# manuelbb-upb/Morbit.jl

Hardware: AMD Instinct MI355X
Metric: RBF build+solve+eval cycles/sec (higher is better)
Workload: dtype f64

## Files before the change

include/mrbf.h:

```cpp
#ifndef MRBF_H
#define MRBF_H

#include <stdint.h>

#ifdef __cplusplus
extern "C" {
#endif

typedef struct mrbf_ctx mrbf_ctx;
typedef struct mrbf_model mrbf_model;

enum {
    MRBF_CUBIC = 0,
    MRBF_INV_MULTIQUADRIC = 1,
    MRBF_MULTIQUADRIC = 2,
    MRBF_THIN_PLATE_SPLINE = 3,
    MRBF_GAUSSIAN = 4
};

enum {
    MRBF_OK = 0,
    MRBF_ENOTPD = 1,
    MRBF_ESINGULAR = 2,
    MRBF_EHIP = 3,
// ... 169 lines not shown

int32_t mrbf_debug_env(const char *name);
int32_t mrbf_debug_mfma_layout(mrbf_ctx *ctx, double *out16x16_a_times_b, const double *A16x4, const double *B4x16);
int32_t mrbf_debug_potrf(mrbf_ctx *ctx, int64_t n, double *A_colmajor_inout, int32_t impl, int32_t *info, float *ms);
int32_t mrbf_debug_diag(mrbf_ctx *ctx, const double *A128, int32_t reps, float *ms_per_call, double *shader_cycles,
                        double *realtime_us);
int32_t mrbf_debug_mfma_peak(mrbf_ctx *ctx, int32_t blocks_per_cu, int32_t threads, int32_t iters, float *ms, double *tflops);
int32_t mrbf_debug_mfma_asm(mrbf_ctx *ctx, int32_t variant, int32_t blocks_per_cu, int32_t iters, float *ms, double *tflops,
                            double *cycles_per_mfma);
int32_t mrbf_debug_dgemm(mrbf_ctx *ctx, int32_t m, int32_t n, int32_t k, float *ms, double *tflops);
int32_t mrbf_debug_mega_tables(int32_t nt, int32_t mt, int32_t slack, int32_t slack_chain, int32_t first, int32_t win, int32_t srows,
                               int32_t half_cols, int64_t *out6);
int32_t mrbf_debug_mega_tables2(int32_t nt, int32_t mt, int32_t slack, int32_t slack_chain, int32_t first, int32_t win, int32_t srows,
                                int32_t half_cols, const int32_t *opt5, int64_t *out6);
int32_t mrbf_debug_mega_plan(int32_t nt, int32_t mt, int32_t xreal, int64_t *out39);

enum { MRBF_PS_OK = 0, MRBF_PS_CRITICAL = 1, MRBF_PS_FAILURE = 2 };
typedef struct {
    int32_t max_ideal_evals;
    int32_t max_ps_evals;
    int32_t max_polish_evals;
    int32_t reserved;
    uint64_t seed;
    double t0;
    double xtol_rel;
} mrbf_ps_options;
typedef struct {
    int32_t status;
    int32_t generations;
    int32_t evals_ideal, evals_ps, evals_polish;
// ... 135 lines not shown
```

morbit.jl_amd/_lib.py:

```python
import ctypes
import os

import numpy as np

_HERE = os.path.dirname(os.path.abspath(__file__))
LIB_PATH = os.environ.get("MRBF_LIB") or os.path.join(_HERE, "libmrbf.so")

c_dp = ctypes.POINTER(ctypes.c_double)
c_fp = ctypes.POINTER(ctypes.c_float)
c_ip = ctypes.POINTER(ctypes.c_int32)
c_vp = ctypes.c_void_p

MRBF_OK, MRBF_ENOTPD, MRBF_ESINGULAR, MRBF_EHIP, MRBF_EBLAS, MRBF_ENOMEM, MRBF_ENODEVICE, MRBF_ENCCL = range(8)
PATH_CHOL, PATH_PROJ_CHOL, PATH_LU, PATH_MINNORM, PATH_ROUND4 = 1, 2, 3, 4, 5
OPT_GRAM_MODE, OPT_RESIDUAL, OPT_FORCE_PATH, OPT_CHOL_IMPL, OPT_EVAL_IMPL, OPT_TIMING, OPT_DIAG_IMPL, OPT_CHOL_WINDOW = 1, 2, 3, 4, 5, 6, 7, 8
OPT_SPIN_MS, OPT_DEBUG_FAULT, OPT_LAST_DEVICE_MS, OPT_SLOW_LAUNCHES = 9, 10, 11, 12
OPT_ARENA_BYTES, OPT_LIVE_HANDLES = 13, 14
FB_CHOL_HOST_DRIVEN, FB_BACKSOLVE_BLOCKED, FB_LU = 1, 2, 4


class FitInfo(ctypes.Structure):
    _fields_ = [("path", ctypes.c_int32), ("factor_info", ctypes.c_int32), ("n", ctypes.c_int32), ("q", ctypes.c_int32),
                ("rel_residual", ctypes.c_double), ("max_pitw", ctypes.c_double), ("mu", ctypes.c_double),
                ("ms_gram", ctypes.c_float), ("ms_project", ctypes.c_float), ("ms_factor", ctypes.c_float),
# ... 167 lines not shown
    "mrbf_batch_run": (ctypes.c_int32, [ctypes.c_int32, c_ip, ctypes.c_int64, ctypes.POINTER(Problem),
                                        ctypes.POINTER(Result)]),
    "mrbf_fit_batch": (ctypes.c_int32, [c_vp, ctypes.c_int64, ctypes.POINTER(FitJob), c_fp]),
    "mrbf_dispatch_fit_batch": (ctypes.c_int32, [ctypes.c_int64]),
    "mrbf_debug_mfma_layout": (ctypes.c_int32, [c_vp, c_vp, c_vp, c_vp]),
    "mrbf_debug_potrf": (ctypes.c_int32, [c_vp, ctypes.c_int64, c_vp, ctypes.c_int32, c_ip, c_fp]),
    "mrbf_debug_env": (ctypes.c_int32, [ctypes.c_char_p]),
    "mrbf_debug_diag": (ctypes.c_int32, [c_vp, c_vp, ctypes.c_int32, c_fp, c_dp, c_dp]),
    "mrbf_debug_ps_rank": (ctypes.c_int32, [c_vp, ctypes.c_int32, c_vp, c_vp, ctypes.c_uint64, ctypes.c_int32, ctypes.c_int32, c_ip, c_ip]),
    "mrbf_debug_mfma_peak": (ctypes.c_int32, [c_vp, ctypes.c_int32, ctypes.c_int32, ctypes.c_int32, c_fp, c_dp]),
    "mrbf_debug_mfma_asm": (ctypes.c_int32, [c_vp, ctypes.c_int32, ctypes.c_int32, ctypes.c_int32, c_fp, c_dp, c_dp]),
    "mrbf_debug_dgemm": (ctypes.c_int32, [c_vp, ctypes.c_int32, ctypes.c_int32, ctypes.c_int32, c_fp, c_dp]),
    "mrbf_debug_mega_tables": (ctypes.c_int32, [ctypes.c_int32] * 8 + [c_vp]),
    "mrbf_debug_mega_tables2": (ctypes.c_int32, [ctypes.c_int32] * 8 + [c_vp, c_vp]),
    "mrbf_debug_mega_plan": (ctypes.c_int32, [ctypes.c_int32] * 3 + [c_vp]),
    "mrbf_stochastic_rank": (ctypes.c_int32, [ctypes.c_int32, c_vp, c_vp, c_vp, ctypes.c_double, c_vp]),
    "mrbf_ps_step": (ctypes.c_int32, [c_vp, c_vp, c_vp, c_vp, c_vp, c_vp, c_vp, ctypes.POINTER(PsOptions), c_vp, c_vp, c_vp,
                                      ctypes.POINTER(PsInfo)]),
    "mrbf_ps_step_problem": (ctypes.c_int32, [c_vp, ctypes.POINTER(PsProblem), c_vp, c_vp, c_vp, c_vp, c_vp, ctypes.POINTER(PsOptions),
                                              c_vp, c_vp, c_vp, ctypes.POINTER(PsInfo)]),
    "mrbf_ps_step_batch": (ctypes.c_int32, [c_vp, ctypes.c_int64, ctypes.POINTER(PsProblem), ctypes.POINTER(ctypes.c_void_p), c_vp, c_vp, c_vp,
                                            c_vp, c_vp, ctypes.POINTER(PsOptions), ctypes.POINTER(ctypes.c_uint64), c_vp, c_vp, c_vp,
                                            ctypes.POINTER(PsInfo), c_fp]),
    "mrbf_dispatch_ps_batch": (ctypes.c_int32, [ctypes.c_int64] + [ctypes.c_int32] * 6),
    "mrbf_sd_direction": (ctypes.c_int32, [c_vp, ctypes.c_int64, ctypes.c_int32, ctypes.c_int32, ctypes.c_int32, ctypes.c_int32] + [c_vp] * 8
                          + [ctypes.c_int32, c_vp, c_vp, c_vp, c_vp, c_vp]),
    "mrbf_sd_criticality": (ctypes.c_int32, [c_vp, ctypes.POINTER(PsProblem), c_vp, c_vp, c_vp, c_vp, ctypes.c_int32, c_vp, c_vp,
                                             ctypes.POINTER(SdInfo)]),
    "mrbf_normal_direction": (ctypes.c_int32, [c_vp, ctypes.c_int64, ctypes.c_int32, ctypes.c_int32, ctypes.c_int32] + [c_vp] * 12),
    "mrbf_normal_step": (ctypes.c_int32, [c_vp, ctypes.POINTER(PsProblem), ctypes.c_int32, c_vp, c_vp, c_vp, ctypes.c_double, ctypes.c_double,
# ... 112 lines not shown
```

morbit.jl_amd/csrc/batch.hip:

```cpp
#include <algorithm>
#include <thread>

#include "common.hpp"
#include "small.hpp"

namespace mrbf {

int batch_run_chain(int n_dev, const int *devs, const std::vector<int64_t> &which, const mrbf_problem *problems, mrbf_result *results);
mrbf_ctx *batch_pool_acquire(int device, int *rc);
void batch_pool_release(mrbf_ctx *c);
void fill_small_prob(const mrbf_ctx *ctx, const mrbf_model *M, const double *Y, double *ws, int *flags, double *scal, int *cl, smallfit::Prob *P);
int small_fit_verdict(const mrbf_model *M, const int *hflags, const double *hscal, mrbf_fit_info *info);
int check_kernel(mrbf_ctx *ctx, int kid, double a, double b, int deg, int argpos);

struct CheckDesc {
    const double *V, *Y;
    const double *C, *Wc, *W;
    const double *vals;
    int64_t n, npad, m;
    int d, k, q;
    double *out;
};

__global__ __launch_bounds__(256) void batch_check_kernel(const CheckDesc *__restrict__ many, int part) {
// ... 103 lines not shown
    if (longest == 0) return 0;
    const unsigned gx = (unsigned)std::min<int64_t>((longest + 2047) / 2048, 256);
    hipLaunchKernelGGL(batch_copy_kernel, dim3(gx, (unsigned)count), dim3(256), 0, ctx->stream, dsegs);
    MRBF_HIP(ctx, hipGetLastError());
    return 0;
}

static int run_small_batch(mrbf_ctx *ctx, const std::vector<int64_t> &idx, const mrbf_problem *problems, mrbf_result *results,
                           std::vector<int64_t> *redo, int force_nc = 0, const mrbf_model *keep = nullptr, float *ms_sum = nullptr) {
    const int P = (int)idx.size();
    if (P == 0) return 0;
    (void)hipSetDevice(ctx->device);
    struct Lay {
        size_t C, Y, X, Xc, sq, mean, W, Wc, lam, ws, Xq0, xsq0, vp0, gp0, V0, Xq1, xsq1, vp1, gp1, vals, jac, out;
        int nsplit0, nsplit1, D, q, KO;
        int64_t npad, mpad0, mpad1;
        bool w_host, lam_host;
    };
    std::vector<Lay> lay(P);
    size_t total = 0;
    auto take = [&](size_t cnt) {
        const size_t at = total;
        total += al16(std::max<size_t>(cnt, 1));
        return at;
    };
    const bool check = ctx->residual != 0;
    const size_t out0 = take((size_t)10 * P);
    for (int i = 0; i < P; ++i) {
        const mrbf_problem &pr = problems[idx[i]];
        Lay &L = lay[i];
// ... 8 lines not shown
        L.X = (pr.m == 0 || is_device_ptr(pr.X)) ? (size_t)-1 : take((size_t)pr.m * d);
        const bool w_dev = pr.weights_out && is_device_ptr(pr.weights_out), lam_dev = pr.poly_out && L.q > 0 && is_device_ptr(pr.poly_out);
        L.w_host = pr.weights_out && !w_dev;
        L.lam_host = pr.poly_out && L.q > 0 && !lam_dev;
        L.Xc = L.sq = L.mean = L.W = L.Wc = L.lam = (size_t)-1;
        if (!keep) {
            L.Xc = take((size_t)L.npad * L.D);
            L.sq = take((size_t)L.npad);
            L.mean = take((size_t)L.D);
            if (!w_dev) L.W = take((size_t)pr.n * k);
            L.Wc = take((size_t)L.npad * k);
            if (!lam_dev) L.lam = take((size_t)std::max(L.q, 1) * k);
        }
        L.ws = take(smallfit::carve((int)L.npad, q16).total);
        L.mpad0 = check ? round_up(pr.n, 64) : 0;
        L.nsplit0 = check ? eval_nsplit(ctx, pr.n, (int)((pr.n + 63) / 64), true) : 1;
        L.Xq0 = take((size_t)L.mpad0 * L.D);
        L.xsq0 = take((size_t)L.mpad0);
        L.vp0 = take(L.nsplit0 > 1 ? (size_t)L.nsplit0 * L.mpad0 * L.KO * 2 : 0);
        L.gp0 = take((size_t)0);
        L.V0 = take((size_t)pr.n * k);
        L.mpad1 = round_up(pr.m, 64);
        L.nsplit1 = pr.m > 0 ? eval_nsplit(ctx, pr.m, (int)((pr.n + 63) / 64)) : 1;
        L.Xq1 = take((size_t)L.mpad1 * L.D);
        L.xsq1 = take((size_t)L.mpad1);
        L.vp1 = take(L.nsplit1 > 1 ? (size_t)L.nsplit1 * L.mpad1 * L.KO * 2 : 0);
        L.gp1 = take((pr.jac_out && L.nsplit1 > 1) ? (size_t)L.nsplit1 * L.mpad1 * L.KO * L.D : 0);
        L.vals = (pr.m == 0 || (pr.vals_out && is_device_ptr(pr.vals_out))) ? (size_t)-1 : take((size_t)pr.m * k);
        L.jac = (pr.m == 0 || !pr.jac_out || is_device_ptr(pr.jac_out)) ? (size_t)-1 : take((size_t)pr.m * k * d);
        L.out = out0 + (size_t)8 * i;
    }
    const size_t arena_budget = (size_t)(mrbf_env("MRBF_BATCH_ARENA_MB") ? atoll(mrbf_env("MRBF_BATCH_ARENA_MB")) : 8192) << 20;
    auto halves = [&]() -> int {
        const std::vector<int64_t> lo(idx.begin(), idx.begin() + P / 2), hi(idx.begin() + P / 2, idx.end());
        MRBF_TRY(run_small_batch(ctx, lo, problems, results, redo, force_nc, keep, ms_sum));
        return run_small_batch(ctx, hi, problems, results, redo, force_nc, keep, ms_sum);
    };
    if (P > 1 && total * sizeof(double) > arena_budget) return halves();
// ... 66 lines not shown
            M.lam = K.lam;
            if (pr.weights_out && !L.w_host) segs[(size_t)P + i] = CopySeg{M.W, pr.weights_out, pr.n * pr.k};
            if (pr.poly_out && L.q > 0 && !L.lam_host) segs[(size_t)2 * P + i] = CopySeg{M.lam, pr.poly_out, (int64_t)L.q * pr.k};
        } else {
            M.Xc = base + L.Xc;
            M.sq = base + L.sq;
            M.mean = base + L.mean;
            M.W = L.W == (size_t)-1 ? pr.weights_out : base + L.W;
            M.Wc = base + L.Wc;
            M.lam = L.lam == (size_t)-1 ? pr.poly_out : base + L.lam;
        }
        fill_small_prob(ctx, &M, Y, base + L.ws, flags + 4 * i, base + L.out + 5, dcl + smallfit::CL_WORDS * i, &probs[i]);
        probs[i].mean_given = 1;
        for (int e = 0; e < 2; ++e) {
            EvalDesc &E = evs[(size_t)e * P + i];
            eval_desc_model(E, &M, e == 0 ? (check ? pr.n : 0) : pr.m, e == 0 ? L.nsplit0 : L.nsplit1);
            E.X = e == 0 ? C : X;
            E.Xq = base + (e == 0 ? L.Xq0 : L.Xq1);
            E.xsq = base + (e == 0 ? L.xsq0 : L.xsq1);
            E.vpart = base + (e == 0 ? L.vp0 : L.vp1);
            E.sapart = E.vpart + (size_t)E.nsplit * E.mpad * L.KO;
            E.gpart = base + (e == 0 ? L.gp0 : L.gp1);
            E.vals = e == 0 ? base + L.V0 : (L.vals == (size_t)-1 ? pr.vals_out : base + L.vals);
            E.jac = e == 0 ? nullptr : (pr.jac_out ? (L.jac == (size_t)-1 ? pr.jac_out : base + L.jac) : nullptr);
        }
        CheckDesc &K = chk[i];
        K.V = base + L.V0;
        K.Y = Y;
        K.C = C;
        K.Wc = M.Wc;
        K.W = M.W;
// ... 356 lines not shown
```

morbit.jl_amd/csrc/batch_chain.hpp:

```cpp
#pragma once
#include "small.hpp"

namespace mrbf {
namespace chain {

struct Arena {
    size_t total = 0;
    size_t take(size_t cnt) {
        const size_t at = total;
        total += (cnt + 15) & ~(size_t)15;
        return at;
    }
};
struct Staging {
    std::vector<double> own;
    double *p;
    Staging(mrbf_ctx *ctx, size_t cnt) {
        p = reinterpret_cast<double *>(cnt * sizeof(double) <= ((size_t)4 << 20) ? pin_take(ctx, cnt * sizeof(double)) : nullptr);
        if (!p) {
            own.resize(cnt);
            p = own.data();
        }
    }
};

constexpr int64_t MAX_GROUP_LAUNCH = 65535;

struct Member {
    int site, j;
    int64_t p;
    int group;
    const mrbf_model *M;
    int64_t mq;
    bool jac;
    size_t X = 0, vals = 0, jacs = 0;
    size_t Xq = 0, xsq = 0, vpart = 0, gpart = 0;
    int64_t mpad = 0;
    int nsplit = 1, KO = 0;
};
struct Group {
    int site, D, k;
    bool jac;
    KP kp;
    std::vector<size_t> members;
    size_t first;
};

struct Plan {
    std::vector<Member> mem;
    std::vector<Group> groups;
    size_t n_desc = 0;

    void add(const mrbf_ctx *ctx, int site, int64_t p, int j, const mrbf_model *M, int64_t mq, bool jac, bool population = false) {
        Member mb;
        mb.site = site, mb.j = j, mb.p = p, mb.M = M, mb.mq = mq, mb.jac = jac;
        mb.nsplit = eval_nsplit(ctx, mq, (int)((M->n + 63) / 64), false, population);
        mb.group = group_of(ctx, site, M, jac, mb.nsplit > 1);
        if (mb.group >= 0) groups[mb.group].members.push_back(mem.size());
        mem.push_back(mb);
    }
    Plan select(const mrbf_ctx *ctx, const std::vector<size_t> &which) const {
        Plan out;
        for (size_t i : which) {
            Member mb = mem[i];
            mb.group = out.group_of(ctx, mb.site, mb.M, mb.jac, mb.nsplit > 1);
            if (mb.group >= 0) out.groups[mb.group].members.push_back(out.mem.size());
            out.mem.push_back(mb);
        }
        out.close();
        return out;
    }
// ... 8 lines not shown
            if (S.group < 0) continue;
            S.mpad = round_up(S.mq, 64);
            S.KO = outputs_per_pass(S.M->k, S.M->dpad, S.jac);
            S.Xq = take((size_t)S.mpad * S.M->dpad);
            S.xsq = take((size_t)S.mpad);
            S.vpart = take(S.nsplit > 1 ? (size_t)S.nsplit * S.mpad * S.KO * 2 : 0);
            S.gpart = take((S.nsplit > 1 && S.jac) ? (size_t)S.nsplit * S.mpad * S.KO * S.M->dpad : 0);
        }
    }
    void fill(double *base, EvalDesc *hdesc) const {
        for (const Group &G : groups)
            for (size_t r = 0; r < G.members.size(); ++r) {
                const Member &S = mem[G.members[r]];
                EvalDesc E;
                std::memset(&E, 0, sizeof(E));
                eval_desc_model(E, S.M, S.mq, S.nsplit);
                E.X = base + S.X;
                E.Xq = base + S.Xq;
                E.xsq = base + S.xsq;
                if (S.nsplit > 1) {
                    E.vpart = base + S.vpart;
                    E.sapart = E.vpart + (size_t)S.nsplit * S.mpad * S.KO;
                    if (S.jac) E.gpart = base + S.gpart;
                }
                E.vals = base + S.vals;
                E.jac = S.jac ? base + S.jacs : nullptr;
                std::memcpy(&hdesc[G.first + r], &E, sizeof(E));
            }
    }
    int launch(mrbf_ctx *ctx, int site, double *base, const EvalDesc *hdesc, const EvalDesc *ddesc, bool centred = false) const {
        for (const Group &G : groups) {
// ... 34 lines not shown
```

morbit.jl_amd/csrc/chol_blocked.hip:

```cpp
#include "common.hpp"
#include "mega_gemm.hpp"

namespace mrbf {

typedef double v4d __attribute__((ext_vector_type(4)));
typedef double v2d __attribute__((ext_vector_type(2)));

constexpr int CNB = 128;

enum { UPD_LOWER_SUB = 0, UPD_OVERWRITE = 1, UPD_FULL_SUB = 2, UPD_COLUMN_SUB = 3 };
int launch_diag_v4(mrbf_ctx *ctx, hipStream_t st, double *Ajj, int64_t lda, double *Linv, int *dinfo, int col0);

template <int TM, int MODE>
__global__ __launch_bounds__(256, 2) void chol_update_kernel(const double *__restrict__ A, int64_t lda,
                                                             const double *__restrict__ B, int64_t ldb,
                                                             double *__restrict__ C, int64_t ldc, int K,
                                                             const int *__restrict__ info, int mt_sq = 0, int ntiles_total = 0,
                                                             const double *__restrict__ cvec = nullptr, double cs = 0.0, int64_t cn = 0) {
    constexpr int NJ = (TM == 128) ? 4 : 2;
    __shared__ __attribute__((aligned(16))) double smem[mega::NSTG * mega::STG];
    if (info && *info != 0) return;
    if (MODE == UPD_OVERWRITE || MODE == UPD_COLUMN_SUB) __builtin_amdgcn_s_setprio(2);
    const int tid = threadIdx.x, lane = tid & 63, wave = tid >> 6;
    const int l15 = lane & 15, l4 = lane >> 4;
    const int tile_end = (MODE == UPD_LOWER_SUB && ntiles_total > 0) ? ntiles_total : (int)blockIdx.x + 1;
    for (int bid = blockIdx.x; bid < tile_end; bid += gridDim.x) {
    int ti, tj;
    if (MODE == UPD_LOWER_SUB) {
        const int ntri = mt_sq * (mt_sq + 1) / 2;
        if (bid < ntri || mt_sq == 0) {
            int t = (int)((sqrt(8.0 * (double)bid + 1.0) - 1.0) * 0.5);
            while ((t + 1) * (t + 2) / 2 <= bid) ++t;
            while (t * (t + 1) / 2 > bid) --t;
            ti = t;
            tj = bid - t * (t + 1) / 2;
        } else {
            ti = mt_sq + (bid - ntri) / mt_sq;
            tj = (bid - ntri) % mt_sq;
        }
    } else {
        ti = blockIdx.x;
        tj = blockIdx.y;
    }
    const int64_t I0 = (int64_t)ti * TM, J0 = (int64_t)tj * 128;
    const int ioff = (TM == 128) ? (wave >> 1) * 64 : 0;
    const int joff = (TM == 128) ? (wave & 1) * 64 : wave * 32;

    v4d acc[NJ][4];
#pragma unroll
    for (int j = 0; j < NJ; ++j)
#pragma unroll
        for (int i = 0; i < 4; ++i) acc[j][i] = (v4d){0.0, 0.0, 0.0, 0.0};

    asm volatile("s_waitcnt vmcnt(0)" ::: "memory");
    constexpr bool NEG_START = (MODE == UPD_LOWER_SUB);
    if (NEG_START) {
#pragma unroll
        for (int j = 0; j < NJ; ++j)
#pragma unroll
// ... 37 lines not shown
        for (int r = 0; r < 4; ++r) {
            const int64_t gj = J0 + joff + j * 16 + l4 + 4 * r;
#pragma unroll
            for (int i = 0; i < 4; ++i) {
                const int64_t gi = I0 + ioff + i * 16 + l15;
                double *dst = C + gi + gj * ldc;
                if (MODE == UPD_OVERWRITE) {
                    *dst = acc[j][i][r];
                } else if (MODE == UPD_FULL_SUB) {
                    *dst = cv[r][i] - acc[j][i][r];
                } else if (MODE == UPD_COLUMN_SUB) {
                    if (gi >= gj) *dst = cv[r][i] - acc[j][i][r];
                } else {
                    double x = -acc[j][i][r];
                    if (cvec) x -= fma(cei[i], cvj[r], cvi[i] * cej[r]);
                    if (ti != tj || gi >= gj) *dst = x;
                }
            }
        }
    }
    if (bid + (int)gridDim.x < tile_end) __syncthreads();
    }
}

struct __attribute__((aligned(16))) DiagShared {
    double col[2][2 * CNB];
    double rinv[2];
    int sbad;
    unsigned long long seg[4];
    int stamp;
};

__device__ __forceinline__ double fast_rsqrt(double x) {
    double y = __builtin_amdgcn_rsq(x);
    const double h = 0.5 * x;
#pragma unroll
// ... 253 lines not shown
    if (const char *e = mrbf_env("MRBF_DIAG_DBG")) {
        if (atoi(e) & 4) {
            double seg[6];
            MRBF_HIP(ctx, hipMemcpy(seg, Linv, sizeof(seg), hipMemcpyDeviceToHost));
            fprintf(stderr, "diag segments (wave 0, cycles over 8 panels): pre-leaf %.0f leaf %.0f post-leaf %.0f wait-X %.0f deferred %.0f wait-Y %.0f\n",
                    seg[0], seg[1], seg[2], seg[3], seg[4], seg[5]);
        }
    }
    MRBF_HIP(ctx, hipMemcpy(stamps_host, st, 6 * sizeof(unsigned long long), hipMemcpyDeviceToHost));
    return 0;
}

int launch_update_lower(mrbf_ctx *ctx, const double *A, int64_t lda, const double *B, int64_t ldb, double *C, int64_t ldc, int64_t nt,
                        int K, const double *cvec, double cs, int64_t cn) {
    if (nt <= 0 || K <= 0) return 0;
    hipLaunchKernelGGL((chol_update_kernel<128, UPD_LOWER_SUB>), dim3((unsigned)(nt * (nt + 1) / 2)), dim3(256), 0, ctx->stream, A,
                       lda, B, ldb, C, ldc, K, (const int *)nullptr, (int)nt, 0, cvec, cs, cn);
    MRBF_HIP(ctx, hipGetLastError());
    return 0;
}

int potrf_blocked_tall(mrbf_ctx *ctx, int64_t ncols, int64_t mrows, double *A, int64_t lda, int *dinfo, double *linv_all, PotrfOpts opt) {
    if (ncols % CNB != 0 || mrows % CNB != 0 || mrows < ncols || (lda & 1) || (reinterpret_cast<uintptr_t>(A) & 15))
        return fail(ctx, MRBF_EHIP, "potrf_blocked needs 128-padded, 16-byte aligned storage (ncols=%lld mrows=%lld lda=%lld)",
                    (long long)ncols, (long long)mrows, (long long)lda);
    const int impl = opt.impl != 0 ? opt.impl : ctx->chol_impl;
    if ((impl == 3 || (impl == 0 && ncols <= ctx->mega.max)) && (opt.any_size || ncols >= ctx->mega.min))
        return potrf_mega_tall(ctx, ncols, mrows, A, lda, dinfo, linv_all, opt);
    double *Lone = nullptr;
    if (!linv_all) MRBF_TRY(get_buf(ctx, S_CHOL_WS, (size_t)CNB * CNB, &Lone));
    hipStream_t S = ctx->stream, M = ctx->bulk_stream, P = ctx->panel_stream;
    hipEvent_t evStart = ctx->evx[0], evT = ctx->evx[1], evU2 = ctx->evx[2], evEnd = ctx->evx[3];
// ... 172 lines not shown
```

morbit.jl_amd/csrc/eval_fused.hip:

```cpp
#include <type_traits>

#include "radial.hpp"
#ifndef MRBF_EVAL_DBG
#define MRBF_EVAL_DBG 0
#endif
#include "small.hpp"

namespace mrbf {

typedef double v4d __attribute__((ext_vector_type(4)));
typedef double v2d __attribute__((ext_vector_type(2)));

constexpr int EQ = 64;
constexpr int EC = 64;

template <int KID, bool FAST, int KOUT, bool JAC, bool FINAL>
__global__ __launch_bounds__(256, 2) void eval_fused_kernel(EvalDesc one, const EvalDesc *__restrict__ many, int l0) {
    constexpr int D = 64, DT = D / 16, LDC = D + 2;
    __shared__ __attribute__((aligned(16))) double Cs[EC * LDC];
    __shared__ double Ws[KOUT * EC];
    __shared__ double Sq[EC];
    const EvalDesc &E = many ? many[blockIdx.z] : one;
    if (many && ((int64_t)blockIdx.x * EQ >= E.mpad || (int)blockIdx.y >= E.nsplit)) return;
    const double *__restrict__ Xq = E.Xq;
// ... 687 lines not shown
    const int D = Dfixed > 0 ? Dfixed : (E.d <= 64 ? 64 : 128);
    const int lane = threadIdx.x & 63;
    const int64_t row = (int64_t)blockIdx.x * (blockDim.x >> 6) + (threadIdx.x >> 6);
    if (row >= E.mpad) return;
    double s = 0.0;
    for (int t = lane; t < D; t += 64) {
        double v = 0.0;
        if (row < E.m && t < E.d) v = E.X[row * E.d + t] - E.mean[t];
        E.Xq[row * D + t] = v;
        s = fma(v, v, s);
    }
    for (int off = 32; off > 0; off >>= 1) s += __shfl_xor(s, off);
    if (lane == 0) E.xsq[row] = s;
}

int eval_nsplit(const mrbf_ctx *ctx, int64_t m, int ntiles, bool check_call, bool population) {
    const int64_t mpad = round_up(m, EQ);
    const int slots = 2 * ctx->ncu;
    const int64_t qtiles = mpad / EQ;
    constexpr int small_split = 8;
    const bool small_batch = !check_call && qtiles * 8 <= slots;
    if (ntiles >= 4 && ntiles <= 8 && small_batch) return std::min(small_split, ntiles);
    if (population && !check_call && ntiles >= 4 && ntiles <= 8 && qtiles * 2 <= slots) return (int)std::min<int64_t>(ntiles, slots / qtiles);
    if (ntiles <= 8) return 1;
    constexpr double comb_small = 0.1, comb = 0.75;
    int nsplit = 1;
    double best_cost = 1e300;
    for (int s = 1; s <= std::min(ntiles, 32); ++s) {
        const int tps_s = (ntiles + s - 1) / s;
        if ((int64_t)(s - 1) * tps_s >= ntiles) continue;
        const double rounds = std::ceil((double)(qtiles * s) / slots);
        const double cost = rounds * tps_s + (small_batch ? comb_small : comb) * s;
        if (cost < best_cost) {
            best_cost = cost;
            nsplit = s;
        }
    }
    const int force_split = mrbf_env("MRBF_EVAL_NSPLIT") ? atoi(mrbf_env("MRBF_EVAL_NSPLIT")) : 0;
    if (force_split > 0 && force_split <= ntiles && (int64_t)(force_split - 1) * ((ntiles + force_split - 1) / force_split) < ntiles)
        nsplit = force_split;
    return nsplit;
}

int outputs_per_pass(int k, int D, bool want_jac) { return (k < 2 || (D == 256 && want_jac)) ? 1 : 2; }

template <int KID, bool FAST, int KOUT, bool JAC, bool FINAL>
static int launch_pass(mrbf_ctx *ctx, int D, dim3 grid, dim3 cgrid, const EvalDesc &one, const EvalDesc *many, int l0) {
    hipStream_t st = ctx->stream;
    if (D == 64) {
        hipLaunchKernelGGL((eval_fused_kernel<KID, FAST, KOUT, JAC, FINAL>), grid, dim3(256), 0, st, one, many, l0);
    } else if (D == 128) {
        hipLaunchKernelGGL((eval_fused_split_kernel<KID, FAST, KOUT, 64, 64, JAC, FINAL>), grid, dim3(512), 0, st, one, many, l0);
    } else if constexpr (JAC && KOUT == 1) {
        hipLaunchKernelGGL((eval_fused_split_kernel<KID, FAST, 1, 128, 32, true, FINAL>), grid, dim3(512), 0, st, one, many, l0);
    } else if constexpr (JAC) {
        return fail(ctx, MRBF_EHIP, "eval_fused: a pass with Jacobians at D = 256 carries one output");
// ... 61 lines not shown
                return fail(ctx, MRBF_EHIP, "eval_fused_batch: descriptor %d is unsplit in a group that splits the centre range", p);
    if (!centred)
        hipLaunchKernelGGL(center_pad_batch_kernel, dim3((unsigned)((max_mpad + 3) / 4), (unsigned)count), dim3(256), 0, ctx->stream, dev_descs, D);
    dim3 grid((unsigned)(max_mpad / EQ), (unsigned)max_split, (unsigned)count);
    dim3 cgrid((unsigned)max_m, (unsigned)count);
    return run_passes(ctx, kp, D, k, want_jac, max_split == 1, grid, cgrid, host_descs[0], dev_descs);
}

int eval_fused(mrbf_ctx *ctx, const mrbf_model *M, int64_t m, const double *X, double *vals, double *jac, mrbf_eval_info *info, EvalHints hints) {
    const int d = M->d, k = M->k;
    const int D = (M->dpad <= 64) ? 64 : (M->dpad <= 128 ? 128 : 256);
    if (M->dpad > 256) return fail(ctx, MRBF_EHIP, "eval_fused supports d <= 256");
    if (D != M->dpad) return fail(ctx, MRBF_EHIP, "eval_fused needs dpad in {64, 128, 256} (got %d)", M->dpad);
    const int64_t mpad = round_up(m, EQ);
    const int ntiles = (int)((M->n + EC - 1) / EC);
    const int nsplit = eval_nsplit(ctx, m, ntiles, hints.check_call, hints.population);
    const int KO = outputs_per_pass(k, D, jac != nullptr);
    EvalDesc E;
    std::memset(&E, 0, sizeof(E));
    eval_desc_model(E, M, m, nsplit);
    E.X = X;
    MRBF_TRY(get_buf(ctx, S_EVAL_XC, (size_t)mpad * D, &E.Xq));
    MRBF_TRY(get_buf(ctx, S_EVAL_XSQ, (size_t)mpad, &E.xsq));
    if (nsplit > 1) {
        MRBF_TRY(get_buf(ctx, S_EVAL_SA, (size_t)nsplit * mpad * KO * 2, &E.vpart));
        E.sapart = E.vpart + (size_t)nsplit * mpad * KO;
        if (jac) MRBF_TRY(get_buf(ctx, S_EVAL_J, (size_t)nsplit * mpad * KO * D, &E.gpart));
    }
    E.vals = vals;
    E.jac = jac;
    const bool timing = ctx->timing && info;
    if (timing) MRBF_HIP(ctx, hipEventRecord(ctx->ev[4], ctx->stream));
    if (!(hints.pre_xq && hints.pre_xq == E.Xq)) MRBF_TRY(launch_center_pad(ctx, X, m, d, M->mean, nullptr, E.Xq, mpad, D, E.xsq));
    dim3 grid((unsigned)(mpad / EQ), (unsigned)nsplit);
    MRBF_TRY(run_passes(ctx, M->kp, D, k, jac != nullptr, nsplit == 1, grid, dim3((unsigned)m), E, nullptr));
    if (timing) {
        MRBF_HIP(ctx, hipEventRecord(ctx->ev[7], ctx->stream));
        MRBF_HIP(ctx, hipEventSynchronize(ctx->ev[7]));
        float t;
        MRBF_HIP(ctx, hipEventElapsedTime(&t, ctx->ev[4], ctx->ev[7]));
        info->ms_total = t;
        info->ms_kernel = t;
    }
    return 0;
}

}
```

morbit.jl_amd/csrc/ps_solver.hip:

```cpp
#include "batch_chain.hpp"
#include "radial.hpp"

namespace mrbf {

namespace ps {

constexpr int MAXLAM = 7168;
constexpr int MAXRUNS = 9;
constexpr int MAXMODELS = 8;
constexpr int MAXOBJ = 8;
constexpr int MAXCON = 32;
constexpr int RANK_THREADS = 1024;
constexpr int RS_B = 256, RS_MINLAM = 1024, RS_CUS_PER_RUN = 16;
constexpr int RS_SYNC = 64;

struct RankWs {
    double *f[2];
    int *idx;
    int *sync;
    int *cnt;
    int *sticky;
};

struct Run {
// ... 1493 lines not shown
    }
    P.nlin_eq = prob->n_lin_eq;
    P.nlin_ineq = prob->n_lin_ineq;
    P.eq_tol = prob->eq_tol >= 0.0 ? prob->eq_tol : 1e-8;
}

static size_t ps_start_doubles(const mrbf_ctx *ctx, const mrbf_model *const *models, int nm, int d, int k, int nftot, bool need_ideal) {
    const size_t lam_ip = 20 * (size_t)(d + 1), lam_ps = 20 * (size_t)(d + 2);
    const size_t rows = std::max(need_ideal ? k * lam_ip : 0, lam_ps);
    const size_t state = std::max(need_ideal ? k * (4 * lam_ip * d + 3 * lam_ip) : 0, 4 * lam_ps * (d + 1) + 3 * lam_ps);
    size_t scratch = 0;
    for (size_t m : {need_ideal ? k * lam_ip : 0, lam_ps}) {
        size_t s = 0;
        for (int j = 0; j < nm && m; ++j) {
            const size_t mpad = (size_t)round_up((int64_t)m, 64);
            const int nsplit = eval_nsplit(ctx, (int64_t)m, (int)((models[j]->n + 63) / 64), false, true);
            s += mpad * (models[j]->dpad + 1) + (nsplit > 1 ? (size_t)nsplit * mpad * 2 * 2 : 0) + 64;
        }
        scratch = std::max(scratch, s);
    }
    return rows * (d + nftot) + state + scratch + 4096;
}

static int ps_step_many(mrbf_ctx *ctx, std::vector<PsStart> &S, bool need_ideal, const mrbf_ps_options *opts, float *ms_out) {
    using namespace ps;
    const size_t N = S.size();
    const bool single = N == 1;
    const Problem &P0 = S[0].P;
    const int d = P0.d, k = P0.nobj, nm = P0.nmodels, nftot = P0.nftot;
    hipStream_t st = ctx->stream;
    hipEvent_t e0 = ctx->ev[0], e1 = ctx->ev[1];
// ... 609 lines not shown
```

morbit.jl_amd/csrc/small.hpp:

```cpp
#pragma once
#include "common.hpp"

namespace mrbf {
namespace smallfit {

struct Prob {
    int n, d, k, q, deg;
    int n16, npad, dpad, q16;
    KP kp;
    const double *C, *Y;
    double *Xc, *sq, *mean, *W, *Wc, *lam;
    double *ws;
    int *flags;
    double *scal;
    long long *stamps;
    int *cl;
    int mean_given;
    unsigned long long spin_ticks;
    int fault;
    int diag6;
};

constexpr int CL_WORDS = 24;
constexpr int MAX_CLUSTER = 16;
// ... 34 lines not shown
}

struct EvalDesc {
    const double *X;
    const double *mean;
    double *Xq, *xsq;
    const double *Cc, *csq, *Wc, *lam;
    int64_t npad, mpad, m;
    int d, k, q, tiles_per_split, nsplit;
    int ntiles;
    int nsub;
    KP kp;
    double *vpart, *sapart, *gpart;
    double *vals, *jac;
};
inline void eval_desc_model(EvalDesc &E, const mrbf_model *M, int64_t m, int nsplit) {
    E.mean = M->mean;
    E.Cc = M->Xc;
    E.csq = M->sq;
    E.Wc = M->Wc;
    E.lam = M->lam;
    E.npad = M->npad;
    E.d = M->d;
    E.k = M->k;
    E.q = M->q;
    E.kp = M->kp;
    E.m = m;
    E.mpad = round_up(m, 64);
    E.nsplit = nsplit;
    E.ntiles = (int)((M->n + 63) / 64);
    E.nsub = (int)((M->n + 15) / 16);
    E.tiles_per_split = (E.ntiles + nsplit - 1) / nsplit;
}
int eval_nsplit(const mrbf_ctx *ctx, int64_t m, int ntiles, bool check_call = false, bool population = false);
int outputs_per_pass(int k, int D, bool want_jac = true);
int eval_fused_batch(mrbf_ctx *ctx, const KP &kp, int D, int k, bool want_jac, const EvalDesc *host_descs, const EvalDesc *dev_descs, int count,
                     bool centred = false);
int center_pad_batch(mrbf_ctx *ctx, const EvalDesc *dev_descs, int count, int64_t max_mpad);

bool small_fit_applies(const mrbf_ctx *ctx, int64_t n, int d, int k, int q, int path);
int launch_small_fit(mrbf_ctx *ctx, const smallfit::Prob *host_probs, int count, const smallfit::Prob *dev_probs, int nc);
int small_fit_cluster(const mrbf_ctx *ctx, int count);
int launch_small_means(mrbf_ctx *ctx, const smallfit::Prob *dev_probs, int count);

bool tail_basis_applies(const mrbf_model *M);
size_t tail_basis_scratch_doubles();
int launch_tail_basis(mrbf_ctx *ctx, const mrbf_model *M, const double *Y, double *scratch, double *LinvX, double *T1, double *Q1, double *B,
                      double *rows_out, int64_t ld, int xt, int *flags);

// ... 2 lines not shown
```

Baseline: 176.1.

## Simulate grid scheduling to choose eval split and split trailing Cholesky update tiles

```diff
diff --git a/include/mrbf.h b/include/mrbf.h
--- a/include/mrbf.h
+++ b/include/mrbf.h
@@ -207,6 +207,8 @@
 int32_t mrbf_debug_mega_tables2(int32_t nt, int32_t mt, int32_t slack, int32_t slack_chain, int32_t first, int32_t win, int32_t srows,
                                 int32_t half_cols, const int32_t *opt5, int64_t *out6);
 int32_t mrbf_debug_mega_plan(int32_t nt, int32_t mt, int32_t xreal, int64_t *out39);
+
+int32_t mrbf_debug_eval_split(int64_t m, int32_t ntiles, int32_t ncu, int32_t *nsplit, int32_t *tiles_per_split);
 
 enum { MRBF_PS_OK = 0, MRBF_PS_CRITICAL = 1, MRBF_PS_FAILURE = 2 };
 typedef struct {
diff --git a/morbit.jl_amd/_lib.py b/morbit.jl_amd/_lib.py
--- a/morbit.jl_amd/_lib.py
+++ b/morbit.jl_amd/_lib.py
@@ -205,6 +205,7 @@
     "mrbf_debug_mega_tables": (ctypes.c_int32, [ctypes.c_int32] * 8 + [c_vp]),
     "mrbf_debug_mega_tables2": (ctypes.c_int32, [ctypes.c_int32] * 8 + [c_vp, c_vp]),
     "mrbf_debug_mega_plan": (ctypes.c_int32, [ctypes.c_int32] * 3 + [c_vp]),
+    "mrbf_debug_eval_split": (ctypes.c_int32, [ctypes.c_int64, ctypes.c_int32, ctypes.c_int32, c_ip, c_ip]),
     "mrbf_stochastic_rank": (ctypes.c_int32, [ctypes.c_int32, c_vp, c_vp, c_vp, ctypes.c_double, c_vp]),
     "mrbf_ps_step": (ctypes.c_int32, [c_vp, c_vp, c_vp, c_vp, c_vp, c_vp, c_vp, ctypes.POINTER(PsOptions), c_vp, c_vp, c_vp,
                                       ctypes.POINTER(PsInfo)]),
diff --git a/morbit.jl_amd/csrc/batch.hip b/morbit.jl_amd/csrc/batch.hip
--- a/morbit.jl_amd/csrc/batch.hip
+++ b/morbit.jl_amd/csrc/batch.hip
@@ -141,6 +141,7 @@
     struct Lay {
         size_t C, Y, X, Xc, sq, mean, W, Wc, lam, ws, Xq0, xsq0, vp0, gp0, V0, Xq1, xsq1, vp1, gp1, vals, jac, out;
         int nsplit0, nsplit1, D, q, KO;
+        EvalSplit split0, split1;
         int64_t npad, mpad0, mpad1;
         bool w_host, lam_host;
     };
@@ -179,14 +180,16 @@
         }
         L.ws = take(smallfit::carve((int)L.npad, q16).total);
         L.mpad0 = check ? round_up(pr.n, 64) : 0;
-        L.nsplit0 = check ? eval_nsplit(ctx, pr.n, (int)((pr.n + 63) / 64), true) : 1;
+        L.split0 = check ? eval_split(ctx, pr.n, (int)((pr.n + 63) / 64), true) : EvalSplit{1, (int)((pr.n + 63) / 64)};
+        L.nsplit0 = L.split0.nsplit;
         L.Xq0 = take((size_t)L.mpad0 * L.D);
         L.xsq0 = take((size_t)L.mpad0);
         L.vp0 = take(L.nsplit0 > 1 ? (size_t)L.nsplit0 * L.mpad0 * L.KO * 2 : 0);
         L.gp0 = take((size_t)0);
         L.V0 = take((size_t)pr.n * k);
         L.mpad1 = round_up(pr.m, 64);
-        L.nsplit1 = pr.m > 0 ? eval_nsplit(ctx, pr.m, (int)((pr.n + 63) / 64)) : 1;
+        L.split1 = pr.m > 0 ? eval_split(ctx, pr.m, (int)((pr.n + 63) / 64)) : EvalSplit{1, (int)((pr.n + 63) / 64)};
+        L.nsplit1 = L.split1.nsplit;
         L.Xq1 = take((size_t)L.mpad1 * L.D);
         L.xsq1 = take((size_t)L.mpad1);
         L.vp1 = take(L.nsplit1 > 1 ? (size_t)L.nsplit1 * L.mpad1 * L.KO * 2 : 0);
@@ -283,7 +286,7 @@
         probs[i].mean_given = 1;
         for (int e = 0; e < 2; ++e) {
             EvalDesc &E = evs[(size_t)e * P + i];
-            eval_desc_model(E, &M, e == 0 ? (check ? pr.n : 0) : pr.m, e == 0 ? L.nsplit0 : L.nsplit1);
+            eval_desc_model(E, &M, e == 0 ? (check ? pr.n : 0) : pr.m, e == 0 ? L.split0 : L.split1);
             E.X = e == 0 ? C : X;
             E.Xq = base + (e == 0 ? L.Xq0 : L.Xq1);
             E.xsq = base + (e == 0 ? L.xsq0 : L.xsq1);
diff --git a/morbit.jl_amd/csrc/batch_chain.hpp b/morbit.jl_amd/csrc/batch_chain.hpp
--- a/morbit.jl_amd/csrc/batch_chain.hpp
+++ b/morbit.jl_amd/csrc/batch_chain.hpp
@@ -37,6 +37,7 @@
     size_t Xq = 0, xsq = 0, vpart = 0, gpart = 0;
     int64_t mpad = 0;
     int nsplit = 1, KO = 0;
+    EvalSplit split;
 };
 struct Group {
     int site, D, k;
@@ -54,7 +55,8 @@
     void add(const mrbf_ctx *ctx, int site, int64_t p, int j, const mrbf_model *M, int64_t mq, bool jac, bool population = false) {
         Member mb;
         mb.site = site, mb.j = j, mb.p = p, mb.M = M, mb.mq = mq, mb.jac = jac;
-        mb.nsplit = eval_nsplit(ctx, mq, (int)((M->n + 63) / 64), false, population);
+        mb.split = eval_split(ctx, mq, (int)((M->n + 63) / 64), false, population);
+        mb.nsplit = mb.split.nsplit;
         mb.group = group_of(ctx, site, M, jac, mb.nsplit > 1);
         if (mb.group >= 0) groups[mb.group].members.push_back(mem.size());
         mem.push_back(mb);
@@ -93,7 +95,7 @@
                 const Member &S = mem[G.members[r]];
                 EvalDesc E;
                 std::memset(&E, 0, sizeof(E));
-                eval_desc_model(E, S.M, S.mq, S.nsplit);
+                eval_desc_model(E, S.M, S.mq, S.split);
                 E.X = base + S.X;
                 E.Xq = base + S.Xq;
                 E.xsq = base + S.xsq;
diff --git a/morbit.jl_amd/csrc/chol_blocked.hip b/morbit.jl_amd/csrc/chol_blocked.hip
--- a/morbit.jl_amd/csrc/chol_blocked.hip
+++ b/morbit.jl_amd/csrc/chol_blocked.hip
@@ -12,37 +12,12 @@
 int launch_diag_v4(mrbf_ctx *ctx, hipStream_t st, double *Ajj, int64_t lda, double *Linv, int *dinfo, int col0);
 
 template <int TM, int MODE>
-__global__ __launch_bounds__(256, 2) void chol_update_kernel(const double *__restrict__ A, int64_t lda,
-                                                             const double *__restrict__ B, int64_t ldb,
-                                                             double *__restrict__ C, int64_t ldc, int K,
-                                                             const int *__restrict__ info, int mt_sq = 0, int ntiles_total = 0,
-                                                             const double *__restrict__ cvec = nullptr, double cs = 0.0, int64_t cn = 0) {
+__device__ __forceinline__ void update_tile(const double *__restrict__ A, int64_t lda, const double *__restrict__ B, int64_t ldb,
+                                            double *__restrict__ C, int64_t ldc, int K, int64_t I0, int64_t J0, bool diag,
+                                            const double *__restrict__ cvec, double cs, int64_t cn, double *smem) {
     constexpr int NJ = (TM == 128) ? 4 : 2;
-    __shared__ __attribute__((aligned(16))) double smem[mega::NSTG * mega::STG];
-    if (info && *info != 0) return;
-    if (MODE == UPD_OVERWRITE || MODE == UPD_COLUMN_SUB) __builtin_amdgcn_s_setprio(2);
     const int tid = threadIdx.x, lane = tid & 63, wave = tid >> 6;
     const int l15 = lane & 15, l4 = lane >> 4;
-    const int tile_end = (MODE == UPD_LOWER_SUB && ntiles_total > 0) ? ntiles_total : (int)blockIdx.x + 1;
-    for (int bid = blockIdx.x; bid < tile_end; bid += gridDim.x) {
-    int ti, tj;
-    if (MODE == UPD_LOWER_SUB) {
-        const int ntri = mt_sq * (mt_sq + 1) / 2;
-        if (bid < ntri || mt_sq == 0) {
-            int t = (int)((sqrt(8.0 * (double)bid + 1.0) - 1.0) * 0.5);
-            while ((t + 1) * (t + 2) / 2 <= bid) ++t;
-            while (t * (t + 1) / 2 > bid) --t;
-            ti = t;
-            tj = bid - t * (t + 1) / 2;
-        } else {
-            ti = mt_sq + (bid - ntri) / mt_sq;
-            tj = (bid - ntri) % mt_sq;
-        }
-    } else {
-        ti = blockIdx.x;
-        tj = blockIdx.y;
-    }
-    const int64_t I0 = (int64_t)ti * TM, J0 = (int64_t)tj * 128;
     const int ioff = (TM == 128) ? (wave >> 1) * 64 : 0;
     const int joff = (TM == 128) ? (wave & 1) * 64 : wave * 32;
 
@@ -110,12 +85,55 @@
                 } else {
                     double x = -acc[j][i][r];
                     if (cvec) x -= fma(cei[i], cvj[r], cvi[i] * cej[r]);
-                    if (ti != tj || gi >= gj) *dst = x;
+                    if (!diag || gi >= gj) *dst = x;
                 }
             }
         }
     }
-    if (bid + (int)gridDim.x < tile_end) __syncthreads();
+}
+
+template <int TM, int MODE>
+__global__ __launch_bounds__(256, 2) void chol_update_kernel(const double *__restrict__ A, int64_t lda,
+                                                             const double *__restrict__ B, int64_t ldb,
+                                                             double *__restrict__ C, int64_t ldc, int K,
+                                                             const int *__restrict__ info, int mt_sq = 0, int ntiles_total = 0,
+                                                             const double *__restrict__ cvec = nullptr, double cs = 0.0, int64_t cn = 0,
+                                                             int ncut = 0) {
+    __shared__ __attribute__((aligned(16))) double smem[mega::NSTG * mega::STG];
+    if (info && *info != 0) return;
+    if (MODE == UPD_OVERWRITE || MODE == UPD_COLUMN_SUB) __builtin_amdgcn_s_setprio(2);
+    const int tile_end = (MODE == UPD_LOWER_SUB && ntiles_total > 0) ? ntiles_total : (int)blockIdx.x + 1;
+    for (int bid = blockIdx.x; bid < tile_end; bid += gridDim.x) {
+        int ti, tj, half = -1;
+        if (MODE == UPD_LOWER_SUB) {
+            int tile = bid;
+            if (TM == 128 && ncut > 0) {
+                const int nwhole = (int)gridDim.x - 2 * ncut;
+                if (bid >= nwhole) {
+                    tile = nwhole + ((bid - nwhole) >> 1);
+                    half = (bid - nwhole) & 1;
+                }
+            }
+            const int ntri = mt_sq * (mt_sq + 1) / 2;
+            if (tile < ntri || mt_sq == 0) {
+                int t = (int)((sqrt(8.0 * (double)tile + 1.0) - 1.0) * 0.5);
+                while ((t + 1) * (t + 2) / 2 <= tile) ++t;
+                while (t * (t + 1) / 2 > tile) --t;
+                ti = t;
+                tj = tile - t * (t + 1) / 2;
+            } else {
+                ti = mt_sq + (tile - ntri) / mt_sq;
+                tj = (tile - ntri) % mt_sq;
+            }
+        } else {
+            ti = blockIdx.x;
+            tj = blockIdx.y;
+        }
+        if (TM == 128 && MODE == UPD_LOWER_SUB && half >= 0)
+            update_tile<64, MODE>(A, lda, B, ldb, C, ldc, K, (int64_t)ti * 128 + 64 * half, (int64_t)tj * 128, ti == tj, cvec, cs, cn, smem);
+        else
+            update_tile<TM, MODE>(A, lda, B, ldb, C, ldc, K, (int64_t)ti * TM, (int64_t)tj * 128, ti == tj, cvec, cs, cn, smem);
+        if (bid + (int)gridDim.x < tile_end) __syncthreads();
     }
 }
 
@@ -399,8 +417,11 @@
 int launch_update_lower(mrbf_ctx *ctx, const double *A, int64_t lda, const double *B, int64_t ldb, double *C, int64_t ldc, int64_t nt,
                         int K, const double *cvec, double cs, int64_t cn) {
     if (nt <= 0 || K <= 0) return 0;
-    hipLaunchKernelGGL((chol_update_kernel<128, UPD_LOWER_SUB>), dim3((unsigned)(nt * (nt + 1) / 2)), dim3(256), 0, ctx->stream, A,
-                       lda, B, ldb, C, ldc, K, (const int *)nullptr, (int)nt, 0, cvec, cs, cn);
+    const int64_t tiles = nt * (nt + 1) / 2, slots = 2 * (int64_t)ctx->ncu;
+    const int64_t rem = tiles > slots ? tiles % slots : 0;
+    const int ncut = (rem > 0 && 2 * rem < slots) ? (int)rem : 0;
+    hipLaunchKernelGGL((chol_update_kernel<128, UPD_LOWER_SUB>), dim3((unsigned)(tiles + ncut)), dim3(256), 0, ctx->stream, A, lda, B, ldb,
+                       C, ldc, K, (const int *)nullptr, (int)nt, 0, cvec, cs, cn, ncut);
     MRBF_HIP(ctx, hipGetLastError());
     return 0;
 }
diff --git a/morbit.jl_amd/csrc/eval_fused.hip b/morbit.jl_amd/csrc/eval_fused.hip
--- a/morbit.jl_amd/csrc/eval_fused.hip
+++ b/morbit.jl_amd/csrc/eval_fused.hip
@@ -725,32 +725,77 @@
     if (lane == 0) E.xsq[row] = s;
 }
 
-int eval_nsplit(const mrbf_ctx *ctx, int64_t m, int ntiles, bool check_call, bool population) {
+static double eval_grid_time(int64_t qtiles, int s, int tps, int ntiles, int slots, double fixed) {
+    struct Free {
+        double t;
+        int64_t cnt;
+    };
+    constexpr int CAP = 40;
+    Free fr[CAP] = {{0.0, (int64_t)slots}};
+    int nfr = 1;
+    double end = 0.0;
+    for (int piece = 0; piece < s; ++piece) {
+        const double cost = fixed + (piece < s - 1 ? tps : ntiles - (s - 1) * tps);
+        int64_t left = qtiles;
+        while (left > 0) {
+            const Free f = fr[0];
+            const int64_t take = std::min(left, f.cnt);
+            if (take == f.cnt) {
+                for (int e = 1; e < nfr; ++e) fr[e - 1] = fr[e];
+                --nfr;
+            } else {
+                fr[0].cnt -= take;
+            }
+            left -= take;
+            const double t = f.t + cost;
+            end = std::max(end, t);
+            int at = nfr;
+            while (at > 0 && fr[at - 1].t > t) --at;
+            if (at > 0 && fr[at - 1].t == t) {
+                fr[at - 1].cnt += take;
+            } else {
+                if (nfr == CAP) return 1e300;
+                for (int e = nfr; e > at; --e) fr[e] = fr[e - 1];
+                fr[at] = Free{t, take};
+                ++nfr;
+            }
+        }
+    }
+    return end;
+}
+
+EvalSplit eval_split_rule(int64_t m, int ntiles, int ncu, bool check_call, bool population, int force_split) {
+    auto even = [&](int s) { return EvalSplit{s, (ntiles + s - 1) / s}; };
     const int64_t mpad = round_up(m, EQ);
-    const int slots = 2 * ctx->ncu;
+    const int slots = 2 * ncu;
     const int64_t qtiles = mpad / EQ;
     constexpr int small_split = 8;
     const bool small_batch = !check_call && qtiles * 8 <= slots;
-    if (ntiles >= 4 && ntiles <= 8 && small_batch) return std::min(small_split, ntiles);
-    if (population && !check_call && ntiles >= 4 && ntiles <= 8 && qtiles * 2 <= slots) return (int)std::min<int64_t>(ntiles, slots / qtiles);
-    if (ntiles <= 8) return 1;
+    if (ntiles >= 4 && ntiles <= 8 && small_batch) return even(std::min(small_split, ntiles));
+    if (population && !check_call && ntiles >= 4 && ntiles <= 8 && qtiles * 2 <= slots) return even((int)std::min<int64_t>(ntiles, slots / qtiles));
+    if (ntiles <= 8) return even(1);
+    if (force_split > 0 && force_split <= ntiles && (int64_t)(force_split - 1) * ((ntiles + force_split - 1) / force_split) < ntiles)
+        return even(force_split);
     constexpr double comb_small = 0.1, comb = 0.75;
-    int nsplit = 1;
+    constexpr double fixed = 1.0;
+    EvalSplit best = even(1);
     double best_cost = 1e300;
-    for (int s = 1; s <= std::min(ntiles, 32); ++s) {
-        const int tps_s = (ntiles + s - 1) / s;
-        if ((int64_t)(s - 1) * tps_s >= ntiles) continue;
-        const double rounds = std::ceil((double)(qtiles * s) / slots);
-        const double cost = rounds * tps_s + (small_batch ? comb_small : comb) * s;
-        if (cost < best_cost) {
-            best_cost = cost;
-            nsplit = s;
-        }
-    }
+    for (int s = 1; s <= std::min(ntiles, 32); ++s)
+        for (int tps = (ntiles + s - 1) / s; tps <= ntiles && (int64_t)(s - 1) * tps < ntiles; ++tps) {
+            const double comb_s = (small_batch ? comb_small : comb) * s;
+            if (fixed + tps + comb_s >= best_cost) break;
+            const double cost = eval_grid_time(qtiles, s, tps, ntiles, slots, fixed) + comb_s;
+            if (cost < best_cost) {
+                best_cost = cost;
+                best = EvalSplit{s, tps};
+            }
+        }
+    return best;
+}
+
+EvalSplit eval_split(const mrbf_ctx *ctx, int64_t m, int ntiles, bool check_call, bool population) {
     const int force_split = mrbf_env("MRBF_EVAL_NSPLIT") ? atoi(mrbf_env("MRBF_EVAL_NSPLIT")) : 0;
-    if (force_split > 0 && force_split <= ntiles && (int64_t)(force_split - 1) * ((ntiles + force_split - 1) / force_split) < ntiles)
-        nsplit = force_split;
-    return nsplit;
+    return eval_split_rule(m, ntiles, ctx->ncu, check_call, population, force_split);
 }
 
 int outputs_per_pass(int k, int D, bool want_jac) { return (k < 2 || (D == 256 && want_jac)) ? 1 : 2; }
@@ -842,11 +887,12 @@
     if (D != M->dpad) return fail(ctx, MRBF_EHIP, "eval_fused needs dpad in {64, 128, 256} (got %d)", M->dpad);
     const int64_t mpad = round_up(m, EQ);
     const int ntiles = (int)((M->n + EC - 1) / EC);
-    const int nsplit = eval_nsplit(ctx, m, ntiles, hints.check_call, hints.population);
+    const EvalSplit split = eval_split(ctx, m, ntiles, hints.check_call, hints.population);
+    const int nsplit = split.nsplit;
     const int KO = outputs_per_pass(k, D, jac != nullptr);
     EvalDesc E;
     std::memset(&E, 0, sizeof(E));
-    eval_desc_model(E, M, m, nsplit);
+    eval_desc_model(E, M, m, split);
     E.X = X;
     MRBF_TRY(get_buf(ctx, S_EVAL_XC, (size_t)mpad * D, &E.Xq));
     MRBF_TRY(get_buf(ctx, S_EVAL_XSQ, (size_t)mpad, &E.xsq));
@@ -874,3 +920,15 @@
 }
 
 }
+
+extern "C" int32_t mrbf_debug_eval_split(int64_t m, int32_t ntiles, int32_t ncu, int32_t *nsplit, int32_t *tiles_per_split) {
+    if (m < 1) return -1;
+    if (ntiles < 1) return -2;
+    if (ncu < 1) return -3;
+    if (!nsplit) return -4;
+    if (!tiles_per_split) return -5;
+    const mrbf::EvalSplit sp = mrbf::eval_split_rule(m, ntiles, ncu, false, false, 0);
+    *nsplit = sp.nsplit;
+    *tiles_per_split = sp.tiles_per_split;
+    return 0;
+}
diff --git a/morbit.jl_amd/csrc/ps_solver.hip b/morbit.jl_amd/csrc/ps_solver.hip
--- a/morbit.jl_amd/csrc/ps_solver.hip
+++ b/morbit.jl_amd/csrc/ps_solver.hip
@@ -1531,7 +1531,7 @@
         size_t s = 0;
         for (int j = 0; j < nm && m; ++j) {
             const size_t mpad = (size_t)round_up((int64_t)m, 64);
-            const int nsplit = eval_nsplit(ctx, (int64_t)m, (int)((models[j]->n + 63) / 64), false, true);
+            const int nsplit = eval_split(ctx, (int64_t)m, (int)((models[j]->n + 63) / 64), false, true).nsplit;
             s += mpad * (models[j]->dpad + 1) + (nsplit > 1 ? (size_t)nsplit * mpad * 2 * 2 : 0) + 64;
         }
         scratch = std::max(scratch, s);
diff --git a/morbit.jl_amd/csrc/small.hpp b/morbit.jl_amd/csrc/small.hpp
--- a/morbit.jl_amd/csrc/small.hpp
+++ b/morbit.jl_amd/csrc/small.hpp
@@ -72,7 +72,10 @@
     double *vpart, *sapart, *gpart;
     double *vals, *jac;
 };
-inline void eval_desc_model(EvalDesc &E, const mrbf_model *M, int64_t m, int nsplit) {
+struct EvalSplit {
+    int nsplit = 1, tiles_per_split = 0;
+};
+inline void eval_desc_model(EvalDesc &E, const mrbf_model *M, int64_t m, EvalSplit split) {
     E.mean = M->mean;
     E.Cc = M->Xc;
     E.csq = M->sq;
@@ -85,12 +88,13 @@
     E.kp = M->kp;
     E.m = m;
     E.mpad = round_up(m, 64);
-    E.nsplit = nsplit;
+    E.nsplit = split.nsplit;
     E.ntiles = (int)((M->n + 63) / 64);
     E.nsub = (int)((M->n + 15) / 16);
-    E.tiles_per_split = (E.ntiles + nsplit - 1) / nsplit;
+    E.tiles_per_split = split.tiles_per_split;
 }
-int eval_nsplit(const mrbf_ctx *ctx, int64_t m, int ntiles, bool check_call = false, bool population = false);
+EvalSplit eval_split(const mrbf_ctx *ctx, int64_t m, int ntiles, bool check_call = false, bool population = false);
+EvalSplit eval_split_rule(int64_t m, int ntiles, int ncu, bool check_call, bool population, int force_split);
 int outputs_per_pass(int k, int D, bool want_jac = true);
 int eval_fused_batch(mrbf_ctx *ctx, const KP &kp, int D, int k, bool want_jac, const EvalDesc *host_descs, const EvalDesc *dev_descs, int count,
                      bool centred = false);
```

Result: no change. 176.0 (-0.0%).
